# GarciaLnk/LlamaRec

Measured on AMD Instinct MI355X. Metric: users/sec through retrieve+rerank, higher is better.
Workload: dtype bf16; 1 GPU; beauty two-stage: LRURec(V=12086, L=50, D=64, 2 blocks) top-50 with history mask -> Llama-2-7b (32 layers, bf16, random init) single prefill -> verbalizer over 20 candidates; batching=token budget 32768 per step (llamarec_amd/packing.py), rmsnorm_folded_into_gemm=False, llama_layers=32, parallelism=dp1, collective_backend=nccl

## Files before the change

### include/llamarec_mi355x.h

```cpp
#ifndef LLAMAREC_MI355X_H
#define LLAMAREC_MI355X_H

#include <stddef.h>
#include <stdint.h>

#ifdef __cplusplus
extern "C" {
#endif

#define LR_OK 0
#define LR_EINVAL (-1)
#define LR_EUNSUPPORTED (-2)
#define LR_EHIP (-3)
#define LR_EWORKSPACE (-4)

#define LR_MAX_LRU_BLOCKS 4
#define LR_MAX_TOPK 64

const char* lr_last_error(void);
const char* lr_version(void);


typedef struct LrLruBlockWeights {
  const float* params_log;
// ... 120 lines not shown
  float final_softcap;
  float attn_scale;
  int32_t reserved[5];
  const uint16_t* const* attn_out_norm;
  const uint16_t* const* mlp_out_norm;
} LrGemma2Ext;
int lr_llama_set_gemma2(lr_llama_t* h, const LrGemma2Ext* ext);

int lr_llama_set_qkv_bias(lr_llama_t* h, const uint16_t* const* bqkv);

int lr_llama_set_qk_norm(lr_llama_t* h, const uint16_t* const* q_norm, const uint16_t* const* k_norm);

int lr_fold_norm_bf16(const uint16_t* w, const uint16_t* norm_w, int32_t rows, int32_t cols, uint16_t* out,
                      void* hip_stream);
int lr_llama_set_folded_norms(lr_llama_t* h, const uint16_t* const* wqkv_folded, const uint16_t* const* wgu_folded);

int lr_llama_set_last_layer_pruning(lr_llama_t* h, int32_t enable);

size_t lr_llama_workspace_bytes(const lr_llama_t* h, int32_t max_tokens, int32_t max_seqs);

int lr_llama_prefill_verbalize(lr_llama_t* h, const int32_t* packed_ids, const int32_t* cu_seqlens,
                               const int32_t* cu_seqlens_host, int32_t B,
                               const int32_t* label_token_ids, int32_t C, float* out_scores,
                               void* workspace, size_t workspace_bytes, void* hip_stream);

int lr_llama_prefill_verbalize_prefix(lr_llama_t* h, const int32_t* packed_ids, const int32_t* cu_seqlens,
                                      const int32_t* cu_seqlens_host, int32_t B, int32_t prefix_len,
                                      const int32_t* label_token_ids, int32_t C, float* out_scores,
                                      void* workspace, size_t workspace_bytes, void* hip_stream);
int32_t lr_common_prefix_len(const int32_t* packed_ids_host, const int32_t* cu_seqlens_host, int32_t B);
// ... 189 lines not shown
```

### llamarec_amd/_lib.py

```python
from __future__ import annotations

import ctypes as C
import os

from . import _abi as A

_HERE = os.path.dirname(os.path.abspath(__file__))
LIB_PATH = os.environ.get("LLAMAREC_LIB") or os.path.join(_HERE, "lib", "libllamarec_mi355x.so")
_lib = None


class LlamaRecError(RuntimeError):
    pass


PROTOTYPES = {
    "lr_last_error": (C.c_char_p, []),
    "lr_version": (C.c_char_p, []),
    "lr_lru_packed_bytes": (C.c_size_t, [C.c_int32, C.c_int32]),
    "lr_lru_pack": (C.c_int, [C.POINTER(A.LrLruWeightsDesc), C.c_void_p, C.c_size_t]),
    "lr_lru_create": (C.c_int, [C.c_void_p, C.c_size_t, C.c_int32, C.c_int32, C.POINTER(C.c_void_p)]),
    "lr_lru_destroy": (None, [C.c_void_p]),
    "lr_lru_set_encoder_pipeline": (C.c_int, [C.c_void_p, C.c_int32]),
    "lr_lru_workspace_bytes": (C.c_size_t, [C.c_void_p, C.c_int32, C.c_int32, C.c_int32]),
# ... 46 lines not shown
    "lr_llama_create_ex": (C.c_int, [C.POINTER(A.LrLlamaConfig), C.POINTER(A.LrLlamaArch), C.POINTER(A.LrLlamaWeightsDesc),
                                     C.POINTER(C.c_void_p)]),
    "lr_llama_destroy": (None, [C.c_void_p]),
    "lr_llama_set_variants": (C.c_int, [C.c_void_p, C.c_int32, C.c_int32]),
    "lr_llama_set_last_layer_pruning": (C.c_int, [C.c_void_p, C.c_int32]),
    "lr_llama_set_rope_scaling": (C.c_int, [C.c_void_p, C.POINTER(A.LrRopeScaling)]),
    "lr_llama_set_gemma2": (C.c_int, [C.c_void_p, C.POINTER(A.LrGemma2Ext)]),
    "lr_llama_set_qkv_bias": (C.c_int, [C.c_void_p, C.c_void_p]),
    "lr_llama_set_qk_norm": (C.c_int, [C.c_void_p, C.c_void_p, C.c_void_p]),
    "lr_qk_norm_rope_bf16": (C.c_int, [C.c_void_p, C.c_int32, C.c_int32, C.c_int32, C.c_int32, C.c_int32, C.c_int32, C.c_void_p,
                                       C.c_void_p, C.c_float, C.c_void_p, C.c_void_p, C.c_void_p]),
    "lr_qk_norm_bwd_bf16": (C.c_int, [C.c_void_p, C.c_int32, C.c_int32, C.c_int32, C.c_void_p, C.c_int32, C.c_int32, C.c_int32,
                                      C.c_int32, C.c_void_p, C.c_void_p, C.c_float, C.c_void_p]),
    "lr_fold_norm_bf16": (C.c_int, [C.c_void_p, C.c_void_p, C.c_int32, C.c_int32, C.c_void_p, C.c_void_p]),
    "lr_llama_set_folded_norms": (C.c_int, [C.c_void_p, C.c_void_p, C.c_void_p]),
    "lr_llama_workspace_bytes": (C.c_size_t, [C.c_void_p, C.c_int32, C.c_int32]),
    "lr_llama_prefill_verbalize": (C.c_int, [C.c_void_p, C.c_void_p, C.c_void_p, C.c_void_p, C.c_int32,
                                             C.c_void_p, C.c_int32, C.c_void_p, C.c_void_p, C.c_size_t,
                                             C.c_void_p]),
    "lr_llama_prefill_verbalize_prefix": (C.c_int, [C.c_void_p, C.c_void_p, C.c_void_p, C.c_void_p, C.c_int32, C.c_int32,
                                                    C.c_void_p, C.c_int32, C.c_void_p, C.c_void_p, C.c_size_t,
                                                    C.c_void_p]),
    "lr_common_prefix_len": (C.c_int32, [C.c_void_p, C.c_void_p, C.c_int32]),
    "lr_llama_last_logits": (C.c_int, [C.c_void_p, C.c_void_p, C.c_void_p, C.c_void_p, C.c_int32,
                                       C.c_void_p, C.c_void_p, C.c_size_t, C.c_void_p]),
    "lr_llama_pack_gate_up": (C.c_int, [C.c_void_p, C.c_void_p, C.c_int32, C.c_int32, C.c_void_p]),
    "lr_llama_pack_qkv": (C.c_int, [C.c_void_p, C.c_void_p, C.c_void_p, C.c_int32, C.c_int32, C.c_int32, C.c_int32,
                                    C.c_void_p]),
    "lr_gemm_bf16_nt": (C.c_int, [C.c_void_p, C.c_void_p, C.c_void_p, C.c_int32, C.c_int32, C.c_int32,
                                  C.c_int32, C.c_void_p]),
# ... 92 lines not shown
```

### llamarec_amd/csrc/api_llama.hip

```cpp
#include <math.h>
#include <stdlib.h>
#include <string.h>

#include <vector>

#include "llama_kernels.h"

typedef unsigned short u16;

extern "C" int lr_llama_create_ex(const LrLlamaConfig* cfg, const LrLlamaArch* arch, const LrLlamaWeightsDesc* w,
                                  lr_llama_t** out) {
  if (!cfg || !w || !out || !w->layers) LR_FAIL(LR_EINVAL, "lr_llama_create: null argument");
  const LrLlamaArch llama_arch = {0, 0, 1.0f, {0, 0, 0, 0, 0}};
  if (!arch) arch = &llama_arch;
  if (arch->norm_style < 0 || arch->norm_style > 1 || arch->mlp_act < 0 || arch->mlp_act > 1 ||
      !(arch->embed_scale > 0.f) || arch->embed_scale != arch->embed_scale)
    LR_FAIL(LR_EINVAL, "lr_llama_create_ex: arch norm_style=%d mlp_act=%d embed_scale=%g", arch->norm_style, arch->mlp_act,
            (double)arch->embed_scale);
  for (int i = 0; i < 5; ++i)
    if (arch->reserved[i]) LR_FAIL(LR_EINVAL, "lr_llama_create_ex: arch reserved word %d is not zero", i);
  if (cfg->num_layers < 1 || cfg->num_heads < 1 || cfg->num_kv_heads < 1 || cfg->vocab_size < 1)
    LR_FAIL(LR_EINVAL, "lr_llama_create: bad config");
  if (cfg->hidden_size % 8 != 0 || cfg->intermediate_size % 16 != 0)
    LR_FAIL(LR_EUNSUPPORTED, "lr_llama_create: hidden_size %% 8 and intermediate_size %% 16 must be 0");
// ... 187 lines not shown
  if (h->q_norm && (wqkv_folded || wgu_folded))
    LR_FAIL(LR_EUNSUPPORTED, "lr_llama_set_folded_norms: not with q/k norms (lr_llama_set_qk_norm)");
  free(h->wqkv_folded);
  free(h->wgu_folded);
  h->wqkv_folded = h->wgu_folded = nullptr;
  if (!wqkv_folded && !wgu_folded) return LR_OK;
  if (!wqkv_folded || !wgu_folded) LR_FAIL(LR_EINVAL, "lr_llama_set_folded_norms: give both arrays or neither");
  const int L = h->cfg.num_layers;
  for (int l = 0; l < L; ++l)
    if (!wqkv_folded[l] || !wgu_folded[l]) LR_FAIL(LR_EINVAL, "lr_llama_set_folded_norms: layer %d has a null matrix", l);
  h->wqkv_folded = (const uint16_t**)malloc(sizeof(void*) * L);
  h->wgu_folded = (const uint16_t**)malloc(sizeof(void*) * L);
  memcpy(h->wqkv_folded, wqkv_folded, sizeof(void*) * L);
  memcpy(h->wgu_folded, wgu_folded, sizeof(void*) * L);
  return LR_OK;
}

struct LlamaWs {
  int32_t *tok_pos, *tok_src, *last_rows, *last_pos, *seg_start;
  float *rope, *rstd;
  u16 *x, *xn, *qkv, *att, *hmid;
  u16 *x_last, *xn_last, *att_last, *h_last, *q_last;
  LrGemmSplitK splitk;
  unsigned* rope16;
  int32_t* prefix_bad;
  void* attn_items;
  size_t attn_items_bytes;
  bool compact;
  size_t total;
};
// ... 110 lines not shown
  if (attn_kernel == LR_ATTN_ROWS256)
    LR_RUN(lr_launch_attn256_items(ws.seg_start, S, n, nh, P, ws.attn_items, ws.attn_items_bytes, st));
  LR_RUN(lr_launch_embed(ids, ws.tok_src, h->embed, c.vocab_size, d, ws.x, n, st, h->arch.embed_scale));
  bool input_normed = false;
#ifdef LR_EXPERIMENTS
  static const bool exp_rstd_once = getenv("LR_EXP_RSTD_ONCE") && getenv("LR_EXP_RSTD_ONCE")[0] == '1';
#define EXP_SKIP_SWEEP (exp_rstd_once && l > 0)
#else
#define EXP_SKIP_SWEEP false
#endif
  for (int l = 0; l < c.num_layers; ++l) {
    const LrLlamaLayerWeights& w = h->layers[l];
    const bool folded = h->wqkv_folded != nullptr;
    const bool last_pruned = l == c.num_layers - 1 && h->prune_last;
    const bool last_q_only = last_pruned && !folded && lr_attention_has_last_row_mode(attn_kernel, hd) && gv != 1;
    if (folded && !EXP_SKIP_SWEEP) LR_RUN(lr_launch_rms_rstd(ws.x, ws.rstd, n, d, c.rms_eps, st));
    if (!folded && !input_normed) LR_RUN(lr_launch_rmsnorm(ws.x, w.input_norm, ws.xn, n, d, c.rms_eps, nullptr, st, ns));
    const int q_w = nh * hd, kv_w = 2 * nkv * hd;
    const u16* const bias = h->bqkv ? h->bqkv[l] : nullptr;
    const u16 *const qn = h->q_norm ? h->q_norm[l] : nullptr, *const kn = h->k_norm ? h->k_norm[l] : nullptr;
    const int epi_qkv = qn ? LR_EPI_STORE : LR_EPI_ROPE;
    if (last_q_only) {
      LR_RUN(lr_launch_gemm({.A = ws.xn, .B = w.wqkv + (size_t)q_w * d, .C = ws.qkv, .M = n, .N = kv_w, .K = d,
                             .epi = epi_qkv, .variant = gv, .rope = qn ? LrGemmRope{} : rope(ws.tok_pos, kv_w / 2),
                             .bias = bias ? bias + q_w : nullptr, .splitk = ws.splitk}, st));
      if (qn) LR_RUN(lr_launch_qk_norm_rope(ws.qkv, n, kv_w, 0, nkv, hd, nullptr, kn, c.rms_eps, ws.tok_pos, ws.rope, st));
      LR_RUN(lr_launch_gather_rows(ws.xn, ws.last_rows, B, d, ws.xn_last, st));
      LR_RUN(lr_launch_gemm({.A = ws.xn_last, .B = w.wqkv, .C = ws.q_last, .M = B, .N = q_w, .K = d, .epi = epi_qkv,
                             .variant = pv, .rope = qn ? LrGemmRope{} : rope(ws.last_pos, q_w), .bias = bias,
                             .splitk = ws.splitk}, st));
      if (qn) LR_RUN(lr_launch_qk_norm_rope(ws.q_last, B, q_w, nh, 0, hd, qn, nullptr, c.rms_eps, ws.last_pos, ws.rope, st));
      LR_RUN(lr_launch_attention_last(ws.qkv, ws.q_last, ws.att_last, attn.cu, attn.cu_host, S, n, nh, nkv, hd, st, P, a_scale,
                                      a_cap));
    } else {
      LR_RUN(lr_launch_gemm({.A = folded ? ws.x : ws.xn, .B = folded ? h->wqkv_folded[l] : w.wqkv, .C = ws.qkv, .M = n,
                             .N = q_w + kv_w, .K = d, .epi = epi_qkv, .variant = gv,
                             .rope = qn ? LrGemmRope{} : rope(ws.tok_pos, q_w + kv_w / 2),
// ... 386 lines not shown
```

### llamarec_amd/csrc/llama_elem.hip

```cpp
#include "llama_kernels.h"
#include "lr_profile.h"

typedef unsigned short u16;
typedef u16 u16x8 __attribute__((ext_vector_type(8)));
typedef float floatx4 __attribute__((ext_vector_type(4)));

__device__ __forceinline__ float block_sum_256(float v, float* red) {
#pragma unroll
  for (int s = 32; s >= 1; s >>= 1) v += __shfl_xor(v, s, 64);
  const int wave = threadIdx.x >> 6, lane = threadIdx.x & 63;
  __syncthreads();
  if (lane == 0) red[wave] = v;
  __syncthreads();
  return red[0] + red[1] + red[2] + red[3];
}

__global__ void token_meta_kernel(const int32_t* cu, int B, int P, int32_t* seg_start, int32_t* tok_pos,
                                  int32_t* tok_src, int32_t* last_rows, int32_t* last_pos, const int32_t* ids,
                                  int32_t* prefix_bad) {
  const int seg = blockIdx.x;
  int start, len, pos0, src0;
  if (P > 0 && seg == 0) {
    start = 0, len = P, pos0 = 0, src0 = cu[0];
  } else {
// ... 529 lines not shown
  const size_t blocks = (total + 255) / 256;
  if (blocks > 0x7fffffffu) LR_FAIL(LR_EUNSUPPORTED, "q/k norm sweep: %d rows exceed the grid limit", rows);
  LrProfScope prof(LR_PROF_ELEMENTWISE, 2.0 * total * 16, st);
#define LR_QKN_CASE(HD)                                                                                                   \
  case HD:                                                                                                                \
    hipLaunchKernelGGL(qk_norm_rope_kernel<HD>, dim3((unsigned)blocks), dim3(256), 0, st, buf, total, per_row, ld, nq,    \
                       q_norm, k_norm, eps, tok_pos, rope_cs);                                                            \
    break;
  switch (hd) {
    LR_QKN_CASE(16) LR_QKN_CASE(32) LR_QKN_CASE(64) LR_QKN_CASE(128) LR_QKN_CASE(256)
  }
#undef LR_QKN_CASE
  LR_CHECK_LAUNCH("qk_norm_rope_kernel");
  return LR_OK;
}
```

### llamarec_amd/csrc/llama_kernels.h

```cpp
#ifndef LLAMA_KERNELS_H
#define LLAMA_KERNELS_H

#include "lr_common.h"
#include "lr_profile.h"

__device__ __forceinline__ float bf2f(unsigned short b) {
  return __builtin_bit_cast(float, (unsigned int)b << 16);
}
__device__ __forceinline__ unsigned short f2bf(float f) {
  return __builtin_bit_cast(unsigned short, (__bf16)f);
}
__device__ __forceinline__ unsigned short swiglu_bf16(float g, float u) {
  float s = bf2f(f2bf(g * __builtin_amdgcn_rcpf(1.0f + __expf(-g))));
  return f2bf(s * u);
}

__device__ __forceinline__ unsigned short geglu_bf16(float g, float u) {
  const float t = tanhf(0.7978845608028654f * (g + 0.044715f * g * g * g));
  float s = bf2f(f2bf(0.5f * g * (1.0f + t)));
  return f2bf(s * u);
}
template <int NS>
__device__ __forceinline__ unsigned short rms_apply(unsigned short w, unsigned short x, float rstd) {
  if (NS == 0) return f2bf(bf2f(w) * bf2f(f2bf(bf2f(x) * rstd)));
// ... 29 lines not shown
int lr_check_rope_scaling(const LrRopeScaling* s, const char* who);
int lr_launch_head(const unsigned short* x, const int32_t* rows ,
                   const unsigned short* norm_w,
                   const unsigned short* lm_head, const int32_t* class_ids, int B, int C, int d, float eps,
                   float* out, int vocab, hipStream_t st,
                   const int32_t* poison = nullptr ,
                   int norm_style = 0,
                   float final_softcap = 0.f );
int lr_launch_residual_postnorm(unsigned short* x, const unsigned short* h, const unsigned short* w_out,
                                const unsigned short* w_next, unsigned short* xn, int rows, int d, float eps, hipStream_t st);
bool lr_qk_norm_head_dim_ok(int hd);
int lr_launch_qk_norm_rope(unsigned short* buf, int rows, int ld, int nq, int nk, int hd, const unsigned short* q_norm,
                           const unsigned short* k_norm, float eps, const int32_t* tok_pos, const float* rope_cs,
                           hipStream_t st);

struct LrGemmRope {
  const int32_t* tok_pos = nullptr;
  const float* cs = nullptr;
  const unsigned* cs16 = nullptr;
  int head_dim = 0, rot_cols = 0;
};
struct LrGemmSplitK { float* ws = nullptr; size_t bytes = 0; };
struct LrGemmThenNorm {
  const unsigned short* w = nullptr;
  unsigned short* out = nullptr;
  float eps = 0.f;
  int style = 0;
  bool* done = nullptr;
};
struct LrGemmArgs {
// ... 189 lines not shown
```

### llamarec_amd/csrc/lr_common.h

```cpp
#ifndef LR_COMMON_H
#define LR_COMMON_H

#include <hip/hip_runtime.h>
#include <stddef.h>
#include <stdint.h>

#include "../../include/llamarec_mi355x.h"
#include "lr_math.h"
#include "lru_topk_plan.h"

void lr_set_error(const char* fmt, ...);
#define LR_FAIL(code, ...)      \
  do {                          \
    lr_set_error(__VA_ARGS__);  \
    return (code);              \
  } while (0)
#define LR_CHECK_HIP(expr)                                                             \
  do {                                                                                 \
    hipError_t e_ = (expr);                                                            \
    if (e_ != hipSuccess) LR_FAIL(LR_EHIP, "%s: %s", #expr, hipGetErrorString(e_));    \
  } while (0)
#define LR_CHECK_LAUNCH(name)                                                          \
  do {                                                                                 \
    hipError_t e_ = hipGetLastError();                                                 \
// ... 115 lines not shown
  LrLlamaLayerWeights* layers;
  int device;
  int gemm_variant;
  int attn_variant;
  int prune_last;
  const uint16_t** wqkv_folded;
  const uint16_t** wgu_folded;
  LrRopeScaling rope_scaling;
  int gemma2;
  float attn_softcap, final_softcap, attn_scale;
  const uint16_t** attn_out_norm;
  const uint16_t** mlp_out_norm;
  const uint16_t** bqkv;
  const uint16_t** q_norm;
  const uint16_t** k_norm;
};

#endif
```

### llamarec_amd/csrc/lr_profile.h

```cpp
#ifndef LR_PROFILE_H
#define LR_PROFILE_H
#include <hip/hip_runtime.h>

#define LR_PROF_GEMM256 0
#define LR_PROF_GEMM_GENERIC 1
#define LR_PROF_ATTN_MFMA 2
#define LR_PROF_ATTN_GENERIC 3
#define LR_PROF_LRU_ENCODE 4
#define LR_PROF_ITEM_TOPK 5
#define LR_PROF_ELEMENTWISE 6

#define LR_PROF_GEMM_TAG(epi, N, K) (((long long)(epi) << 56) | ((long long)(N) << 28) | (long long)(K))
bool lr_prof_begin(int kind, double work, hipStream_t st, long long tag = 0);
void lr_prof_end(hipStream_t st);

struct LrProfScope {
  hipStream_t st;
  bool on;
  LrProfScope(int kind, double work, hipStream_t s, long long tag = 0) : st(s), on(lr_prof_begin(kind, work, s, tag)) {}
  ~LrProfScope() {
    if (on) lr_prof_end(st);
  }
};
#endif
```

### llamarec_amd/llm.py

```python
from __future__ import annotations

import ctypes as C
import json
import os
import re
from dataclasses import dataclass

import numpy as np
import torch

from . import _abi as A
from ._lib import check, lib, stream_ptr

LLAMA2_7B = dict(vocab_size=32000, hidden_size=4096, intermediate_size=11008, num_hidden_layers=32,
                 num_attention_heads=32, num_key_value_heads=32, max_position_embeddings=4096,
                 rms_norm_eps=1e-5, rope_theta=10000.0)
LLAMA3_ROPE_SCALING = dict(rope_type="llama3", factor=32.0, low_freq_factor=1.0, high_freq_factor=4.0,
                           original_max_position_embeddings=8192)
LLAMA32_1B = dict(model_type="llama", vocab_size=128256, hidden_size=2048, intermediate_size=8192, num_hidden_layers=16,
                  num_attention_heads=32, num_key_value_heads=8, head_dim=64, max_position_embeddings=131072,
                  rms_norm_eps=1e-5, rope_theta=500000.0, tie_word_embeddings=True, rope_scaling=dict(LLAMA3_ROPE_SCALING))
LLAMA32_3B = dict(LLAMA32_1B, hidden_size=3072, num_hidden_layers=28, num_attention_heads=24, head_dim=128)
LLAMA31_8B = dict(LLAMA32_1B, hidden_size=4096, intermediate_size=14336, num_hidden_layers=32, num_attention_heads=32,
                  head_dim=128, tie_word_embeddings=False, rope_scaling=dict(LLAMA3_ROPE_SCALING, factor=8.0))
# ... 30 lines not shown
QWEN3_4B = dict(QWEN3_0_6B, hidden_size=2560, intermediate_size=9728, num_hidden_layers=36, num_attention_heads=32,
                max_window_layers=36)
QWEN3_8B = dict(QWEN3_4B, hidden_size=4096, intermediate_size=12288, tie_word_embeddings=False)

LLAMA_FAMILY = ("llama", "mistral")
GEMMA_FAMILY = ("gemma",)
GEMMA2_FAMILY = ("gemma2",)
PHI3_FAMILY = ("phi3",)
QWEN2_FAMILY = ("qwen2",)
QWEN3_FAMILY = ("qwen3",)
SUPPORTED_MODEL_TYPES = LLAMA_FAMILY + PHI3_FAMILY + QWEN2_FAMILY + QWEN3_FAMILY + GEMMA_FAMILY + GEMMA2_FAMILY
GEMMA2_REQUIRED_KEYS = ("query_pre_attn_scalar", "attn_logit_softcapping", "final_logit_softcapping", "sliding_window", "head_dim")
PHI3_REQUIRED_KEYS = ("hidden_act", "original_max_position_embeddings", "sliding_window")
QWEN2_REQUIRED_KEYS = ("hidden_act", "use_sliding_window", "sliding_window", "max_window_layers")
QWEN3_REQUIRED_KEYS = ("head_dim", "hidden_act", "attention_bias")


_LLAMA3_NUMBERS = ("factor", "low_freq_factor", "high_freq_factor", "original_max_position_embeddings")


def rope_parameters(config: dict):
    rp = config.get("rope_parameters")
    rs = config.get("rope_scaling")
    theta = config.get("rope_theta")
    if theta is None and isinstance(rp, dict):
        theta = rp.get("rope_theta")
    src = rs if rs is not None else rp
    if src is None:
        return float(theta if theta is not None else 10000.0), None
    kind = (src.get("rope_type") or src.get("type") or "default") if isinstance(src, dict) else src
# ... 255 lines not shown


def load_peft_adapter(adapter_path):
    from safetensors import safe_open

    r, alpha, modules = check_adapter_config(json.load(open(os.path.join(adapter_path, "adapter_config.json"))))
    t = {}
    with safe_open(os.path.join(adapter_path, "adapter_model.safetensors"), framework="pt", device="cpu") as f:
        for k in f.keys():
            t[k] = f.get_tensor(k).float().numpy()
    return dict(r=r, alpha=alpha, weights=adapter_weights(t, r, modules), target_modules=modules)


class LlamaRanker:

    def __init__(self, config: dict, device="cuda:0"):
        self.config = dict(config)
        self.device = torch.device(device)
        c = self.config
        self.family = model_family(c)
        self.rope_theta, self.rope_scaling = rope_parameters(c)
        self.hd = c.get("head_dim") or c["hidden_size"] // c["num_attention_heads"]
        windowed = (c.get("model_type") == "mistral" or self.family in ("gemma2", "phi3")
                    or (self.family == "qwen2" and c["use_sliding_window"]))
        self.max_prompt_len = c.get("sliding_window") if windowed else None
        self._window_owner = {"gemma2": "Gemma-2", "phi3": "Phi-3", "qwen2": "Qwen2"}.get(self.family, "Mistral")
        self._h = C.c_void_p()
        self._tensors = {}
        self._ws = None
        self._layers_arr = None
        self._folded_arr = None
        self.fold_norms = False
        self.training = False
        self.default_gemm_variant = 6 if self.family == "qwen2" else 0

    @classmethod
    def from_state_dict(cls, state_dict, config, device="cuda:0", lora=None, nf4=False):
        self = cls(config, device)
        dev = self.device
        scratch = {}

        def nf4_roundtrip(w):
            w = w.to(torch.bfloat16).contiguous()
            need = lib().lr_nf4_scratch_bytes(w.numel())
            if scratch.get("n", 0) < need:
                scratch["buf"], scratch["n"] = torch.empty(need, dtype=torch.uint8, device=dev), need
            with torch.cuda.device(dev):
                check(lib().lr_nf4_roundtrip_bf16(w.data_ptr(), w.numel(), 1, w.data_ptr(), scratch["buf"].data_ptr(),
                                                  scratch["n"], stream_ptr()), "lr_nf4_roundtrip_bf16")
            return w

        def t(name):
            w = state_dict[name]
# ... 75 lines not shown
                    T[f"{i}.{n}_norm"] = self._interleave_rope_rows(wn).reshape(-1).to(torch.bfloat16).contiguous()
            T[f"{i}.wo"] = merged(p + "self_attn.o_proj.weight").to(torch.bfloat16).contiguous()
            T[f"{i}.wgu"] = self._interleave_gate_up(gate, up)
            T[f"{i}.wdown"] = merged(p + "mlp.down_proj.weight").to(torch.bfloat16).contiguous()
            T[f"{i}.input_norm"] = t(p + "input_layernorm.weight").to(torch.bfloat16).contiguous()
            if self.family == "gemma2":
                T[f"{i}.post_norm"] = t(p + "pre_feedforward_layernorm.weight").to(torch.bfloat16).contiguous()
                T[f"{i}.attn_out_norm"] = t(p + "post_attention_layernorm.weight").to(torch.bfloat16).contiguous()
                T[f"{i}.mlp_out_norm"] = t(p + "post_feedforward_layernorm.weight").to(torch.bfloat16).contiguous()
            else:
                T[f"{i}.post_norm"] = t(p + "post_attention_layernorm.weight").to(torch.bfloat16).contiguous()
        self._create()
        return self

    @classmethod
    def random_init(cls, config, seed=42, std=0.02, device="cuda:0"):
        self = cls(config, device)
        c, dev = self.config, self.device
        g = torch.Generator(device=dev)
        g.manual_seed(seed)
        d, f, v = c["hidden_size"], c["intermediate_size"], c["vocab_size"]
        nh, nkv, hd = c["num_attention_heads"], c["num_key_value_heads"], self.hd

        def rnd(*shape):
            return (torch.randn(*shape, generator=g, device=dev, dtype=torch.float32) * std).to(torch.bfloat16)

        T = self._tensors
        gemma = self.family in ("gemma", "gemma2")
        norm = torch.zeros if gemma else torch.ones
        T["embed"] = rnd(v, d)
        T["final_norm"] = norm(d, dtype=torch.bfloat16, device=dev)
        T["lm_head"] = T["embed"] if gemma else rnd(v, d)
# ... 4 lines not shown
            if self.family == "qwen3":
                T[f"{i}.q_norm"] = norm(hd, dtype=torch.bfloat16, device=dev)
                T[f"{i}.k_norm"] = norm(hd, dtype=torch.bfloat16, device=dev)
            T[f"{i}.wo"] = rnd(d, nh * hd)
            T[f"{i}.wgu"] = rnd(2 * f, d)
            T[f"{i}.wdown"] = rnd(d, f)
            T[f"{i}.input_norm"] = norm(d, dtype=torch.bfloat16, device=dev)
            T[f"{i}.post_norm"] = norm(d, dtype=torch.bfloat16, device=dev)
            if self.family == "gemma2":
                T[f"{i}.attn_out_norm"] = norm(d, dtype=torch.bfloat16, device=dev)
                T[f"{i}.mlp_out_norm"] = norm(d, dtype=torch.bfloat16, device=dev)
        self._create()
        return self

    @classmethod
    def from_pretrained(cls, path, device="cuda:0", adapter_path=None, load_in_4bit=False):
        from safetensors import safe_open

        cfg = json.load(open(os.path.join(path, "config.json")))
        model_family(cfg)
        sd = {}
        for fn in sorted(os.listdir(path)):
            if fn.endswith(".safetensors"):
                with safe_open(os.path.join(path, fn), framework="pt", device="cpu") as f:
                    for k in f.keys():
                        sd[k] = f.get_tensor(k)
        return cls.from_state_dict(sd, cfg, device, load_peft_adapter(adapter_path) if adapter_path else None,
                                   nf4=load_in_4bit)

    def _interleave_rope_rows(self, w):
        hd = self.hd
        heads = w.shape[0] // hd
        return w.view(heads, 2, hd // 2, w.shape[1]).transpose(1, 2).reshape(heads * hd, w.shape[1])

    @staticmethod
    def _interleave_gate_up(gate, up):
        f, d = gate.shape
        if f % 16:
            raise ValueError("intermediate_size must be a multiple of 16")
        g = gate.to(torch.bfloat16).view(f // 16, 16, d)
        u = up.to(torch.bfloat16).view(f // 16, 16, d)
        return torch.stack([g, u], dim=1).reshape(2 * f, d).contiguous()

# ... 31 lines not shown
            check(lib().lr_llama_set_rope_scaling(self._h, C.byref(words)), "lr_llama_set_rope_scaling")
        if self.family == "gemma2":
            ext, self._gemma2_arrs = self.gemma2_ext()
            check(lib().lr_llama_set_gemma2(self._h, C.byref(ext)), "lr_llama_set_gemma2")
        if "0.bqkv" in T:
            self._bqkv_arr = (C.c_void_p * L)(*[T[f"{i}.bqkv"].data_ptr() for i in range(L)])
            check(lib().lr_llama_set_qkv_bias(self._h, self._bqkv_arr), "lr_llama_set_qkv_bias")
        if "0.q_norm" in T:
            self._qk_norm_arrs = ((C.c_void_p * L)(*[T[f"{i}.q_norm"].data_ptr() for i in range(L)]),
                                  (C.c_void_p * L)(*[T[f"{i}.k_norm"].data_ptr() for i in range(L)]))
            check(lib().lr_llama_set_qk_norm(self._h, *self._qk_norm_arrs), "lr_llama_set_qk_norm")
        if self.default_gemm_variant:
            self.set_variants(gemm=self.default_gemm_variant)
        if self.fold_norms:
            self.set_fold_norms(True)

    def gemma2_ext(self):
        c, T, L = self.config, self._tensors, self.config["num_hidden_layers"]
        ext = A.LrGemma2Ext(attn_softcap=float(c["attn_logit_softcapping"] or 0.0),
                            final_softcap=float(c["final_logit_softcapping"] or 0.0),
                            attn_scale=float(c["query_pre_attn_scalar"]) ** -0.5)
        arrs = None
        if "0.attn_out_norm" in T:
            arrs = ((C.c_void_p * L)(*[T[f"{i}.attn_out_norm"].data_ptr() for i in range(L)]),
                    (C.c_void_p * L)(*[T[f"{i}.mlp_out_norm"].data_ptr() for i in range(L)]))
            ext.attn_out_norm, ext.mlp_out_norm = arrs
        return ext, arrs

    def set_fold_norms(self, enable=True):
        T, L = self._tensors, self.config["num_hidden_layers"]
        if enable and self.family in ("gemma", "gemma2"):
            raise NotImplementedError("folded norms: Gemma's (1 + w) RMSNorm cannot be folded into bf16 weights at HF's rounding")
        if enable and self.family == "qwen2":
            raise NotImplementedError("folded norms: not with Qwen2's q/k/v biases (lr_llama_set_qkv_bias)")
        if enable and self.family == "qwen3":
            raise NotImplementedError("folded norms: not with Qwen3's q/k norms (lr_llama_set_qk_norm)")
        if not enable:
            check(lib().lr_llama_set_folded_norms(self._h, None, None), "lr_llama_set_folded_norms")
            for i in range(L):
                T.pop(f"{i}.wqkv_folded", None)
                T.pop(f"{i}.wgu_folded", None)
            self._folded_arr = None
            self.fold_norms = False
            return self
        qa, ga = (C.c_void_p * L)(), (C.c_void_p * L)()
        with torch.cuda.device(self.device):
            for i in range(L):
                for name, norm, arr in (("wqkv", "input_norm", qa), ("wgu", "post_norm", ga)):
                    w = T[f"{i}.{name}"]
                    out = torch.empty_like(w)
                    check(lib().lr_fold_norm_bf16(w.data_ptr(), T[f"{i}.{norm}"].data_ptr(), w.shape[0], w.shape[1],
                                                  out.data_ptr(), stream_ptr()), "lr_fold_norm_bf16")
                    T[f"{i}.{name}_folded"] = out
                    arr[i] = out.data_ptr()
            torch.cuda.synchronize()
            check(lib().lr_llama_set_folded_norms(self._h, qa, ga), "lr_llama_set_folded_norms")
        self._folded_arr = (qa, ga)
        self.fold_norms = True
        return self

    def set_variants(self, gemm=0, attention=0):
        check(lib().lr_llama_set_variants(self._h, gemm, attention), "lr_llama_set_variants")
        return self

    def set_last_layer_pruning(self, enable=True):
        check(lib().lr_llama_set_last_layer_pruning(self._h, int(bool(enable))), "lr_llama_set_last_layer_pruning")
        return self

    def eval(self):
        return self

    def __del__(self):
        try:
# ... 60 lines not shown
```

### llamarec_amd/rank_train.py

```python
from __future__ import annotations

import ctypes as C
import json
import math
import os
import re
import shutil

import numpy as np
import torch

from . import _abi as A
from ._lib import check, lib, stream_ptr
from .llm import LORA_MODULE_BLOCK, LlamaRanker, expand_target_modules, pack_prompts

IGNORE = -100
PEFT_KEY = "base_model.model.model.layers.{l}.{block}.{p}_proj.lora_{ab}.weight"
DEFAULT_TARGET_MODULES = ("q_proj", "v_proj")


def peft_key(layer, module, ab):
    return PEFT_KEY.format(l=layer, block=LORA_MODULE_BLOCK[module], p=module[:-len("_proj")], ab=ab)


# ... 295 lines not shown
                if mod == "q_proj":
                    add_(w[:nq], rk._interleave_rope_rows(delta(mod)))
                elif mod == "k_proj":
                    add_(w[nq:nq + nkv], rk._interleave_rope_rows(delta(mod)))
                elif mod == "v_proj":
                    add_(w[nq + nkv:], delta(mod))
                elif mod == "o_proj":
                    add_(rk._tensors[f"{l}.wo"], delta(mod))
                elif mod == "down_proj":
                    add_(rk._tensors[f"{l}.wdown"], delta(mod))
                else:
                    gu = rk._tensors[f"{l}.wgu"].view(f // 16, 2, 16, -1)
                    add_(gu[:, 0 if mod == "gate_proj" else 1], delta(mod).view(f // 16, 16, -1))
        if rk.fold_norms:
            rk.set_fold_norms(True)
        self.merged = True
        return rk

    def __del__(self):
        try:
            if self._h.value:
                lib().lr_llama_lora_destroy(self._h)
        except Exception:
            pass


class LLMTrainSamples:

    def __init__(self, args, u2seq, text_dict, tokenizer, prompter=None, rng=None):
        from . import prompt as P
# ... 299 lines not shown
```

Measured before the change: 159.9 users/s.

## Precompute layer-0 QKV per vocab token and gather with RoPE at prefill

Layer 0's QKV projection depends only on the token id, since it is the embedding followed by RMSNorm and the QKV GEMM. This change builds a vocab-by-QKV-width bf16 table once from the weights. At prefill it replaces layer 0's RMSNorm and QKV GEMM with a per-token row gather plus a RoPE rotation kernel. The aim is to remove one layer's QKV GEMM work, at the cost of a large resident table (hundreds of MB for Llama-2-7b) and a memory-bound gather. The table is rebuilt whenever the weights, folding or LoRA merge change.

```diff
diff --git a/include/llamarec_mi355x.h b/include/llamarec_mi355x.h
--- a/include/llamarec_mi355x.h
+++ b/include/llamarec_mi355x.h
@@ -158,6 +158,16 @@
 int lr_fold_norm_bf16(const uint16_t* w, const uint16_t* norm_w, int32_t rows, int32_t cols, uint16_t* out,
                       void* hip_stream);
 int lr_llama_set_folded_norms(lr_llama_t* h, const uint16_t* const* wqkv_folded, const uint16_t* const* wgu_folded);
+
+size_t lr_llama_qkv0_table_bytes(const lr_llama_t* h);
+size_t lr_llama_qkv0_scratch_bytes(const lr_llama_t* h);
+int lr_llama_build_qkv0_table(lr_llama_t* h, uint16_t* table, size_t table_bytes, void* scratch, size_t scratch_bytes,
+                              void* hip_stream);
+int lr_llama_set_qkv0_table(lr_llama_t* h, const uint16_t* table);
+int32_t lr_llama_qkv0_table_in_use(const lr_llama_t* h);
+int lr_qkv0_gather_rope_bf16(const uint16_t* table, int32_t vocab, const int32_t* ids, const int32_t* tok_pos,
+                             const float* rope_cs, int32_t rope_positions, uint16_t* out, int32_t rows, int32_t row_width,
+                             int32_t rot_cols, int32_t head_dim, void* hip_stream);
 
 int lr_llama_set_last_layer_pruning(lr_llama_t* h, int32_t enable);
 
diff --git a/llamarec_amd/_lib.py b/llamarec_amd/_lib.py
--- a/llamarec_amd/_lib.py
+++ b/llamarec_amd/_lib.py
@@ -84,6 +84,13 @@
                                       C.c_int32, C.c_void_p, C.c_void_p, C.c_float, C.c_void_p]),
     "lr_fold_norm_bf16": (C.c_int, [C.c_void_p, C.c_void_p, C.c_int32, C.c_int32, C.c_void_p, C.c_void_p]),
     "lr_llama_set_folded_norms": (C.c_int, [C.c_void_p, C.c_void_p, C.c_void_p]),
+    "lr_llama_qkv0_table_bytes": (C.c_size_t, [C.c_void_p]),
+    "lr_llama_qkv0_scratch_bytes": (C.c_size_t, [C.c_void_p]),
+    "lr_llama_build_qkv0_table": (C.c_int, [C.c_void_p, C.c_void_p, C.c_size_t, C.c_void_p, C.c_size_t, C.c_void_p]),
+    "lr_llama_set_qkv0_table": (C.c_int, [C.c_void_p, C.c_void_p]),
+    "lr_llama_qkv0_table_in_use": (C.c_int32, [C.c_void_p]),
+    "lr_qkv0_gather_rope_bf16": (C.c_int, [C.c_void_p, C.c_int32, C.c_void_p, C.c_void_p, C.c_void_p, C.c_int32, C.c_void_p,
+                                           C.c_int32, C.c_int32, C.c_int32, C.c_int32, C.c_void_p]),
     "lr_llama_workspace_bytes": (C.c_size_t, [C.c_void_p, C.c_int32, C.c_int32]),
     "lr_llama_prefill_verbalize": (C.c_int, [C.c_void_p, C.c_void_p, C.c_void_p, C.c_void_p, C.c_int32,
                                              C.c_void_p, C.c_int32, C.c_void_p, C.c_void_p, C.c_size_t,
diff --git a/llamarec_amd/csrc/api_llama.hip b/llamarec_amd/csrc/api_llama.hip
--- a/llamarec_amd/csrc/api_llama.hip
+++ b/llamarec_amd/csrc/api_llama.hip
@@ -225,6 +225,86 @@
   memcpy(h->wqkv_folded, wqkv_folded, sizeof(void*) * L);
   memcpy(h->wgu_folded, wgu_folded, sizeof(void*) * L);
   return LR_OK;
+}
+
+#define LR_QKV0_CHUNK 4096
+static size_t qkv0_row_width(const lr_llama* h) {
+  return (size_t)(h->cfg.num_heads + 2 * h->cfg.num_kv_heads) * h->cfg.head_dim;
+}
+static bool qkv0_applicable(const lr_llama* h) { return h && h->cfg.head_dim % 8 == 0 && !h->q_norm; }
+static bool qkv0_table_usable(const lr_llama* h) {
+  if (!h->qkv0_table || !qkv0_applicable(h) || h->wqkv_folded || h->gemm_variant == 5) return false;
+  if (h->cfg.num_layers == 1 && h->prune_last) return false;
+  return h->qkv0_built.table == h->qkv0_table && h->qkv0_built.embed == h->embed &&
+         h->qkv0_built.input_norm == h->layers[0].input_norm && h->qkv0_built.wqkv == h->layers[0].wqkv &&
+         h->qkv0_built.bias == (h->bqkv ? h->bqkv[0] : nullptr);
+}
+
+extern "C" size_t lr_llama_qkv0_table_bytes(const lr_llama_t* h) {
+  return qkv0_applicable(h) ? (size_t)h->cfg.vocab_size * qkv0_row_width(h) * sizeof(u16) : 0;
+}
+
+static size_t qkv0_scratch(const lr_llama* h, int32_t** ids, u16** x, u16** xn, char* base) {
+  const size_t chunk = (size_t)(h->cfg.vocab_size < LR_QKV0_CHUNK ? h->cfg.vocab_size : LR_QKV0_CHUNK);
+  const size_t row = lr_align_up(chunk * h->cfg.hidden_size * sizeof(u16), 256);
+  const size_t idb = lr_align_up((size_t)h->cfg.vocab_size * sizeof(int32_t), 256);
+  if (ids) *ids = (int32_t*)base, *x = (u16*)(base + idb), *xn = (u16*)(base + idb + row);
+  return idb + 2 * row;
+}
+
+extern "C" size_t lr_llama_qkv0_scratch_bytes(const lr_llama_t* h) {
+  return qkv0_applicable(h) ? qkv0_scratch(h, nullptr, nullptr, nullptr, nullptr) : 0;
+}
+
+extern "C" int lr_llama_build_qkv0_table(lr_llama_t* h, uint16_t* table, size_t table_bytes, void* scratch,
+                                         size_t scratch_bytes, void* hip_stream) {
+  if (!h || !table || !scratch) LR_FAIL(LR_EINVAL, "lr_llama_build_qkv0_table: null argument");
+  if (!qkv0_applicable(h))
+    LR_FAIL(LR_EUNSUPPORTED, "lr_llama_build_qkv0_table: head_dim %d (a multiple of 8)%s", h->cfg.head_dim,
+            h->q_norm ? ", and the handle has q/k norms (lr_llama_set_qk_norm)" : "");
+  if ((reinterpret_cast<uintptr_t>(table) | reinterpret_cast<uintptr_t>(scratch)) & 255)
+    LR_FAIL(LR_EINVAL, "lr_llama_build_qkv0_table: table and scratch must be 256-byte aligned");
+  const size_t need = lr_llama_qkv0_table_bytes(h), need_scratch = lr_llama_qkv0_scratch_bytes(h);
+  if (table_bytes < need) LR_FAIL(LR_EWORKSPACE, "lr_llama_build_qkv0_table: the table needs %zu bytes, have %zu", need, table_bytes);
+  if (scratch_bytes < need_scratch)
+    LR_FAIL(LR_EWORKSPACE, "lr_llama_build_qkv0_table: the scratch needs %zu bytes, have %zu", need_scratch, scratch_bytes);
+  hipStream_t st = (hipStream_t)hip_stream;
+  const LrLlamaConfig& c = h->cfg;
+  const LrLlamaLayerWeights& w = h->layers[0];
+  const u16* const bias = h->bqkv ? h->bqkv[0] : nullptr;
+  const int d = c.hidden_size, qkv_w = (int)qkv0_row_width(h);
+  const int variant = h->gemm_variant == 5 ? 0 : h->gemm_variant;
+  int32_t* ids;
+  u16 *x, *xn;
+  qkv0_scratch(h, &ids, &x, &xn, (char*)scratch);
+  h->qkv0_built.table = nullptr;
+  LR_RUN(lr_launch_iota(ids, c.vocab_size, 0, st));
+  for (int c0 = 0; c0 < c.vocab_size; c0 += LR_QKV0_CHUNK) {
+    const int rows = c.vocab_size - c0 < LR_QKV0_CHUNK ? c.vocab_size - c0 : LR_QKV0_CHUNK;
+    LR_RUN(lr_launch_embed(ids + c0, nullptr, h->embed, c.vocab_size, d, x, rows, st, h->arch.embed_scale));
+    LR_RUN(lr_launch_rmsnorm(x, w.input_norm, xn, rows, d, c.rms_eps, nullptr, st, h->arch.norm_style));
+    LR_RUN(lr_launch_gemm({.A = xn, .B = w.wqkv, .C = table + (size_t)c0 * qkv_w, .M = rows, .N = qkv_w, .K = d,
+                           .epi = LR_EPI_STORE, .variant = variant, .bias = bias}, st));
+  }
+  h->qkv0_built = {table, h->embed, w.input_norm, w.wqkv, bias};
+  return LR_OK;
+}
+
+extern "C" int lr_llama_set_qkv0_table(lr_llama_t* h, const uint16_t* table) {
+  if (!h) LR_FAIL(LR_EINVAL, "lr_llama_set_qkv0_table: null handle");
+  if (table && table != h->qkv0_built.table)
+    LR_FAIL(LR_EINVAL, "lr_llama_set_qkv0_table: not the table this handle's last lr_llama_build_qkv0_table filled");
+  h->qkv0_table = table;
+  return LR_OK;
+}
+
+extern "C" int32_t lr_llama_qkv0_table_in_use(const lr_llama_t* h) { return h && qkv0_table_usable(h) ? 1 : 0; }
+
+extern "C" int lr_qkv0_gather_rope_bf16(const uint16_t* table, int32_t vocab, const int32_t* ids, const int32_t* tok_pos,
+                                        const float* rope_cs, int32_t rope_positions, uint16_t* out, int32_t rows,
+                                        int32_t row_width, int32_t rot_cols, int32_t head_dim, void* hip_stream) {
+  return lr_launch_qkv0_gather_rope(table, vocab, ids, nullptr, tok_pos, rope_cs, rope_positions, out, rows, row_width,
+                                    rot_cols, head_dim, (hipStream_t)hip_stream);
 }
 
 struct LlamaWs {
@@ -365,13 +445,18 @@
     const bool folded = h->wqkv_folded != nullptr;
     const bool last_pruned = l == c.num_layers - 1 && h->prune_last;
     const bool last_q_only = last_pruned && !folded && lr_attention_has_last_row_mode(attn_kernel, hd) && gv != 1;
+    const bool from_table = l == 0 && qkv0_table_usable(h);
     if (folded && !EXP_SKIP_SWEEP) LR_RUN(lr_launch_rms_rstd(ws.x, ws.rstd, n, d, c.rms_eps, st));
-    if (!folded && !input_normed) LR_RUN(lr_launch_rmsnorm(ws.x, w.input_norm, ws.xn, n, d, c.rms_eps, nullptr, st, ns));
+    if (!folded && !input_normed && !from_table)
+      LR_RUN(lr_launch_rmsnorm(ws.x, w.input_norm, ws.xn, n, d, c.rms_eps, nullptr, st, ns));
     const int q_w = nh * hd, kv_w = 2 * nkv * hd;
     const u16* const bias = h->bqkv ? h->bqkv[l] : nullptr;
     const u16 *const qn = h->q_norm ? h->q_norm[l] : nullptr, *const kn = h->k_norm ? h->k_norm[l] : nullptr;
     const int epi_qkv = qn ? LR_EPI_STORE : LR_EPI_ROPE;
-    if (last_q_only) {
+    if (from_table) {
+      LR_RUN(lr_launch_qkv0_gather_rope(h->qkv0_table, c.vocab_size, ids, ws.tok_src, ws.tok_pos, ws.rope, plan.maxT, ws.qkv, n,
+                                        q_w + kv_w, q_w + kv_w / 2, hd, st));
+    } else if (last_q_only) {
       LR_RUN(lr_launch_gemm({.A = ws.xn, .B = w.wqkv + (size_t)q_w * d, .C = ws.qkv, .M = n, .N = kv_w, .K = d,
                              .epi = epi_qkv, .variant = gv, .rope = qn ? LrGemmRope{} : rope(ws.tok_pos, kv_w / 2),
                              .bias = bias ? bias + q_w : nullptr, .splitk = ws.splitk}, st));
diff --git a/llamarec_amd/csrc/llama_elem.hip b/llamarec_amd/csrc/llama_elem.hip
--- a/llamarec_amd/csrc/llama_elem.hip
+++ b/llamarec_amd/csrc/llama_elem.hip
@@ -567,3 +567,76 @@
   LR_CHECK_LAUNCH("qk_norm_rope_kernel");
   return LR_OK;
 }
+
+template <int HD>
+__global__ __launch_bounds__(256) void qkv0_gather_rope_kernel(const u16* __restrict__ table, int vocab, const int32_t* ids,
+                                                               const int32_t* tok_src, const int32_t* tok_pos,
+                                                               const float* __restrict__ rope_cs, int rope_rows,
+                                                               u16* __restrict__ out, int row_w, int rot_cols, int hd_arg) {
+  const int hd = HD ? HD : hd_arg;
+  const int m = blockIdx.x;
+  int id = ids[tok_src ? tok_src[m] : m];
+  if (id < 0 || id >= vocab) id = 0;
+  int pos = tok_pos[m];
+  pos = pos < 0 ? 0 : (pos >= rope_rows ? rope_rows - 1 : pos);
+  const u16x8* src = reinterpret_cast<const u16x8*>(table + (size_t)id * row_w);
+  u16x8* dst = reinterpret_cast<u16x8*>(out + (size_t)m * row_w);
+  const float* cs = rope_cs + (size_t)pos * hd;
+  const int nv = row_w / 8, nrot = rot_cols / 8;
+  for (int i = threadIdx.x; i < nv; i += 256) {
+    const u16x8 v = src[i];
+    if (i < nrot) {
+      const int i0 = ((i * 8) % hd) >> 1;
+      const float4 t0 = *reinterpret_cast<const float4*>(cs + i0 * 2), t1 = *reinterpret_cast<const float4*>(cs + i0 * 2 + 4);
+      const float co[4] = {t0.x, t0.z, t1.x, t1.z}, si[4] = {t0.y, t0.w, t1.y, t1.w};
+      u16x8 o;
+#pragma unroll
+      for (int q = 0; q < 4; ++q) {
+        const float x0 = bf2f(v[2 * q]), x1 = bf2f(v[2 * q + 1]);
+        o[2 * q] = f2bf(x0 * co[q] - x1 * si[q]);
+        o[2 * q + 1] = f2bf(x1 * co[q] + x0 * si[q]);
+      }
+      dst[i] = o;
+    } else {
+      dst[i] = v;
+    }
+  }
+}
+
+int lr_launch_qkv0_gather_rope(const u16* table, int vocab, const int32_t* ids, const int32_t* tok_src, const int32_t* tok_pos,
+                               const float* rope_cs, int rope_rows, u16* out, int rows, int row_w, int rot_cols, int hd,
+                               hipStream_t st) {
+  if (rows <= 0) return LR_OK;
+  if (!table || !ids || !tok_pos || !rope_cs || !out || vocab < 1 || rope_rows < 1 || hd < 8 || hd % 8 != 0 || row_w < 8 ||
+      row_w % 8 != 0 || rot_cols < 0 || rot_cols > row_w || rot_cols % hd != 0 ||
+      ((reinterpret_cast<uintptr_t>(table) | reinterpret_cast<uintptr_t>(out) | reinterpret_cast<uintptr_t>(rope_cs)) & 15))
+    LR_FAIL(LR_EINVAL, "qkv0 gather: bad argument (vocab %d, rope rows %d, head_dim %d a multiple of 8, row width %d, %d rotated "
+            "columns in whole heads; 16-byte aligned pointers)", vocab, rope_rows, hd, row_w, rot_cols);
+  LrProfScope prof(LR_PROF_QKV0_GATHER, 2.0 * rows * row_w * 2, st);
+#define LR_QKV0_CASE(HD)                                                                                                  \
+  case HD:                                                                                                                \
+    hipLaunchKernelGGL(qkv0_gather_rope_kernel<HD>, dim3(rows), dim3(256), 0, st, table, vocab, ids, tok_src, tok_pos,    \
+                       rope_cs, rope_rows, out, row_w, rot_cols, hd);                                                     \
+    break;
+  switch (hd) {
+    LR_QKV0_CASE(64) LR_QKV0_CASE(96) LR_QKV0_CASE(128) LR_QKV0_CASE(256)
+    default:
+      hipLaunchKernelGGL(qkv0_gather_rope_kernel<0>, dim3(rows), dim3(256), 0, st, table, vocab, ids, tok_src, tok_pos, rope_cs,
+                         rope_rows, out, row_w, rot_cols, hd);
+  }
+#undef LR_QKV0_CASE
+  LR_CHECK_LAUNCH("qkv0_gather_rope_kernel");
+  return LR_OK;
+}
+
+__global__ __launch_bounds__(256) void iota_kernel(int32_t* out, int n, int first) {
+  const int i = blockIdx.x * 256 + threadIdx.x;
+  if (i < n) out[i] = first + i;
+}
+
+int lr_launch_iota(int32_t* out, int n, int first, hipStream_t st) {
+  if (n <= 0) return LR_OK;
+  hipLaunchKernelGGL(iota_kernel, dim3((n + 255) / 256), dim3(256), 0, st, out, n, first);
+  LR_CHECK_LAUNCH("iota_kernel");
+  return LR_OK;
+}
diff --git a/llamarec_amd/csrc/llama_kernels.h b/llamarec_amd/csrc/llama_kernels.h
--- a/llamarec_amd/csrc/llama_kernels.h
+++ b/llamarec_amd/csrc/llama_kernels.h
@@ -67,6 +67,11 @@
                            const unsigned short* k_norm, float eps, const int32_t* tok_pos, const float* rope_cs,
                            hipStream_t st);
 
+int lr_launch_qkv0_gather_rope(const unsigned short* table, int vocab, const int32_t* ids, const int32_t* tok_src,
+                               const int32_t* tok_pos, const float* rope_cs, int rope_rows, unsigned short* out, int rows,
+                               int row_w, int rot_cols, int hd, hipStream_t st);
+int lr_launch_iota(int32_t* out, int n, int first, hipStream_t st);
+
 struct LrGemmRope {
   const int32_t* tok_pos = nullptr;
   const float* cs = nullptr;
diff --git a/llamarec_amd/csrc/lr_common.h b/llamarec_amd/csrc/lr_common.h
--- a/llamarec_amd/csrc/lr_common.h
+++ b/llamarec_amd/csrc/lr_common.h
@@ -153,6 +153,10 @@
   const uint16_t** bqkv;
   const uint16_t** q_norm;
   const uint16_t** k_norm;
+  const uint16_t* qkv0_table;
+  struct {
+    const uint16_t *table, *embed, *input_norm, *wqkv, *bias;
+  } qkv0_built;
 };
 
 #endif
diff --git a/llamarec_amd/csrc/lr_profile.h b/llamarec_amd/csrc/lr_profile.h
--- a/llamarec_amd/csrc/lr_profile.h
+++ b/llamarec_amd/csrc/lr_profile.h
@@ -9,6 +9,7 @@
 #define LR_PROF_LRU_ENCODE 4
 #define LR_PROF_ITEM_TOPK 5
 #define LR_PROF_ELEMENTWISE 6
+#define LR_PROF_QKV0_GATHER 7
 
 #define LR_PROF_GEMM_TAG(epi, N, K) (((long long)(epi) << 56) | ((long long)(N) << 28) | (long long)(K))
 bool lr_prof_begin(int kind, double work, hipStream_t st, long long tag = 0);
diff --git a/llamarec_amd/llm.py b/llamarec_amd/llm.py
--- a/llamarec_amd/llm.py
+++ b/llamarec_amd/llm.py
@@ -68,6 +68,8 @@
 PHI3_REQUIRED_KEYS = ("hidden_act", "original_max_position_embeddings", "sliding_window")
 QWEN2_REQUIRED_KEYS = ("hidden_act", "use_sliding_window", "sliding_window", "max_window_layers")
 QWEN3_REQUIRED_KEYS = ("head_dim", "hidden_act", "attention_bias")
+QKV0_TABLE_MAX_BYTES = 4 << 30
+QKV0_TABLE_MIN_BYTES = 16 << 20
 
 
 _LLAMA3_NUMBERS = ("factor", "low_freq_factor", "high_freq_factor", "original_max_position_embeddings")
@@ -353,9 +355,14 @@
 
 class LlamaRanker:
 
-    def __init__(self, config: dict, device="cuda:0"):
+    def __init__(self, config: dict, device="cuda:0", qkv0_table_max_bytes=QKV0_TABLE_MAX_BYTES,
+                 qkv0_table_min_bytes=QKV0_TABLE_MIN_BYTES):
         self.config = dict(config)
         self.device = torch.device(device)
+        self.qkv0_table_max_bytes = int(qkv0_table_max_bytes)
+        self.qkv0_table_min_bytes = int(qkv0_table_min_bytes)
+        self._qkv0_table = None
+        self.qkv0_table_build_ms = None
         c = self.config
         self.family = model_family(c)
         self.rope_theta, self.rope_scaling = rope_parameters(c)
@@ -374,8 +381,9 @@
         self.default_gemm_variant = 6 if self.family == "qwen2" else 0
 
     @classmethod
-    def from_state_dict(cls, state_dict, config, device="cuda:0", lora=None, nf4=False):
-        self = cls(config, device)
+    def from_state_dict(cls, state_dict, config, device="cuda:0", lora=None, nf4=False,
+                        qkv0_table_max_bytes=QKV0_TABLE_MAX_BYTES, qkv0_table_min_bytes=QKV0_TABLE_MIN_BYTES):
+        self = cls(config, device, qkv0_table_max_bytes, qkv0_table_min_bytes)
         dev = self.device
         scratch = {}
 
@@ -481,8 +489,9 @@
         return self
 
     @classmethod
-    def random_init(cls, config, seed=42, std=0.02, device="cuda:0"):
-        self = cls(config, device)
+    def random_init(cls, config, seed=42, std=0.02, device="cuda:0", qkv0_table_max_bytes=QKV0_TABLE_MAX_BYTES,
+                    qkv0_table_min_bytes=QKV0_TABLE_MIN_BYTES):
+        self = cls(config, device, qkv0_table_max_bytes, qkv0_table_min_bytes)
         c, dev = self.config, self.device
         g = torch.Generator(device=dev)
         g.manual_seed(seed)
@@ -517,7 +526,8 @@
         return self
 
     @classmethod
-    def from_pretrained(cls, path, device="cuda:0", adapter_path=None, load_in_4bit=False):
+    def from_pretrained(cls, path, device="cuda:0", adapter_path=None, load_in_4bit=False,
+                        qkv0_table_max_bytes=QKV0_TABLE_MAX_BYTES, qkv0_table_min_bytes=QKV0_TABLE_MIN_BYTES):
         from safetensors import safe_open
 
         cfg = json.load(open(os.path.join(path, "config.json")))
@@ -529,7 +539,8 @@
                     for k in f.keys():
                         sd[k] = f.get_tensor(k)
         return cls.from_state_dict(sd, cfg, device, load_peft_adapter(adapter_path) if adapter_path else None,
-                                   nf4=load_in_4bit)
+                                   nf4=load_in_4bit, qkv0_table_max_bytes=qkv0_table_max_bytes,
+                                   qkv0_table_min_bytes=qkv0_table_min_bytes)
 
     def _interleave_rope_rows(self, w):
         hd = self.hd
@@ -591,6 +602,35 @@
             self.set_variants(gemm=self.default_gemm_variant)
         if self.fold_norms:
             self.set_fold_norms(True)
+        else:
+            self._refresh_qkv0_table()
+
+    def _refresh_qkv0_table(self):
+        L = lib()
+        check(L.lr_llama_set_qkv0_table(self._h, None), "lr_llama_set_qkv0_table")
+        self._qkv0_table = None
+        self.qkv0_table_build_ms = None
+        if self.fold_norms or os.environ.get("LLAMAREC_QKV0_TABLE", "1") == "0":
+            return
+        need = L.lr_llama_qkv0_table_bytes(self._h)
+        if need == 0 or need > self.qkv0_table_max_bytes or need < self.qkv0_table_min_bytes:
+            return
+        with torch.cuda.device(self.device):
+            table = torch.empty(need, dtype=torch.uint8, device=self.device)
+            scratch = torch.empty(L.lr_llama_qkv0_scratch_bytes(self._h), dtype=torch.uint8, device=self.device)
+            t0, t1 = torch.cuda.Event(enable_timing=True), torch.cuda.Event(enable_timing=True)
+            t0.record()
+            check(L.lr_llama_build_qkv0_table(self._h, table.data_ptr(), table.numel(), scratch.data_ptr(), scratch.numel(),
+                                              stream_ptr()), "lr_llama_build_qkv0_table")
+            t1.record()
+            torch.cuda.synchronize()
+            check(L.lr_llama_set_qkv0_table(self._h, table.data_ptr()), "lr_llama_set_qkv0_table")
+            self.qkv0_table_build_ms = t0.elapsed_time(t1)
+        self._qkv0_table = table
+
+    @property
+    def qkv0_table_in_use(self):
+        return bool(lib().lr_llama_qkv0_table_in_use(self._h))
 
     def gemma2_ext(self):
         c, T, L = self.config, self._tensors, self.config["num_hidden_layers"]
@@ -619,6 +659,7 @@
                 T.pop(f"{i}.wgu_folded", None)
             self._folded_arr = None
             self.fold_norms = False
+            self._refresh_qkv0_table()
             return self
         qa, ga = (C.c_void_p * L)(), (C.c_void_p * L)()
         with torch.cuda.device(self.device):
@@ -634,6 +675,7 @@
             check(lib().lr_llama_set_folded_norms(self._h, qa, ga), "lr_llama_set_folded_norms")
         self._folded_arr = (qa, ga)
         self.fold_norms = True
+        self._refresh_qkv0_table()
         return self
 
     def set_variants(self, gemm=0, attention=0):
diff --git a/llamarec_amd/rank_train.py b/llamarec_amd/rank_train.py
--- a/llamarec_amd/rank_train.py
+++ b/llamarec_amd/rank_train.py
@@ -333,6 +333,8 @@
                     add_(gu[:, 0 if mod == "gate_proj" else 1], delta(mod).view(f // 16, 16, -1))
         if rk.fold_norms:
             rk.set_fold_norms(True)
+        else:
+            rk._refresh_qkv0_table()
         self.merged = True
         return rk
 
```

After: 160.9 users/s (median of 6 runs). No clear change (+0.7%).
